# simplew4y/VeritasFi

Hardware: AMD Instinct MI355X
Metric: queries/sec top-100 over 10Mx768 corpus (higher is better)
Workload: dtype f16

## Files before the change

veritasfi_amd/csrc/vf_api.hip:

```cpp
#include "../../include/veritasfi_hip.h"
#include "vf_internal.h"
#include "vf_route.h"

#include <fcntl.h>
#include <float.h>
#include <sys/stat.h>
#include <unistd.h>
#include <math.h>
#include <string.h>

#include <algorithm>
#include <atomic>
#include <mutex>
#include <string>
#include <vector>

using namespace vf;

static thread_local std::string g_err;

static int fail(int code, const std::string& msg) {
    g_err = msg;
    return code;
}
// ... 40 lines not shown
        bytes = need;
        return VF_OK;
    }
    void release() { if (p) (void)hipFree(p); p = nullptr; bytes = 0; }
    template <class T> T* as() const { return (T*)p; }
};

struct HostBuf {
    void* p = nullptr;
    size_t bytes = 0;
    int ensure(size_t need) {
        if (need <= bytes) return VF_OK;
        if (p) { (void)hipHostFree(p); p = nullptr; bytes = 0; }
        hipError_t e = hipHostMalloc(&p, need, hipHostMallocDefault);
        if (e != hipSuccess) return fail(VF_ENOMEM, std::string("hipHostMalloc(") + std::to_string(need) + "): " + hipGetErrorString(e));
        bytes = need;
        return VF_OK;
    }
    void release() { if (p) (void)hipHostFree(p); p = nullptr; bytes = 0; }
};

struct Slot {
    hipStream_t stream = nullptr;
    hipStream_t scan_stream = nullptr;
    hipEvent_t ev_pro = nullptr;
    hipEvent_t ev_in = nullptr, ev_done = nullptr, ev_scan = nullptr;
    hipEvent_t ev_t[4] = {nullptr, nullptr, nullptr, nullptr};
    bool timed = false;
    int wide_launches = 0, wide_queries = 0;
    int scan_kernel = 0;
    int scan_image = 0;
    DevBuf qn, qimg, s0, cnt, tau, hist, hist_coarse, cand, flags, counts;
    DevBuf dbg, wgbase, tilecnt, sib;
    DevBuf qimg8, epsq;
    DevBuf qscale, bandq;
    int image_i8 = 0;
    int64_t wgbase_n = -1; int wgbase_grid = -1;
    DevBuf dense_s, cn_tmp, parts_ids, parts_sc, run_ids, run_sc, qsel;
    int* h_flags = nullptr;
    u32* h_counts = nullptr;
    int* d_flags = nullptr;
    u32* d_counts = nullptr;
    size_t h_cap = 0;
    bool pending = false;
    const float* d_queries = nullptr;
    int nq = 0, k = 0, path = 0;
    int64_t* d_ids = nullptr;
    float* d_scores = nullptr;
    hipStream_t user_stream = nullptr;
};

struct GroupSlot {
    std::vector<hipStream_t> feed;
    std::vector<hipEvent_t> ev;
    std::vector<DevBuf> dq, blob;
    DevBuf all;
    hipEvent_t ev_in = nullptr;
    hipStream_t hq_stream = nullptr;
    hipEvent_t ev_hq = nullptr;
    HostBuf hq;
    std::vector<hipStream_t> hfeed;
    std::vector<hipEvent_t> ev_hb;
    std::vector<hipEvent_t> ev_home;
    std::vector<HostBuf> hb;
    std::vector<char> staged_last;
    bool pending = false;
    int nq = 0, k = 0;
    int64_t* d_ids = nullptr; float* d_scores = nullptr;
    hipStream_t user = nullptr;
};

}

struct vf_index {
    int device = 0;
    int64_t n = 0;
    int64_t cap = 0;
    int d = 0, dp = 0, dtype = 0;
    int64_t id_offset = 0;
    int n_cu = 256;
    int64_t aux_applied = -1;
    bool owns_rows = false;
    void* rows_orig = nullptr;
    void* rows_scan = nullptr;
    bool owns_scan = false;
    float* norm = nullptr;
    float* inv_scan = nullptr;
    float* cn_cache = nullptr;
    unsigned char* rows_img = nullptr;
    bool owns_img = false;
    float* inv_img = nullptr;
    float rho_max = 0.0f;
    float rho_mean = 0.0f;
    bool image_refused = false;
    float rho_sum = 0.0f;
    std::mutex mu;
    Slot slots[kSlots];
    int64_t force_path = -1, sample_rows = -1, margin = -1, cap_opt = 0, waves_opt = 0, scan_g = 0,
            refresh_every = 128, debug = 0, steal_opt = 0, wide_opt = 1, wide_sync = -1, wide_mfma = -1, wide8_waves = 8, wide8_stage = 0,
            aux_cus = -1, sample_grid = -1, overlap_scans = -1, scan_impl = 2, sample_impl = -1, scan_image = 1, wide_rows = 1, image_mfma = -1;
    vf_search_stats stats{};
    bool profile = false;
    double prof_scan_ms = 0.0, prof_pipe_ms = 0.0;
    int64_t prof_launches = 0, prof_bytes = 0;
    hipEvent_t ev_span = nullptr;
    bool span_started = false;
    bool span_slot[4] = {false, false, false, false};
    DevBuf st_q, st_ids, st_sc;
    DevBuf st_add, st_rho;
    DevBuf st_cmp, st_rem;
    int64_t compact_chunk_rows = 0;
    int64_t subset_super_rows = 0;
    bool damaged = false;
    std::vector<vf_index*> shards;
    std::vector<int> peer_ok;
    GroupSlot gslots[kSlots];
};

static int ensure_pinned(Slot& s, size_t nq_total) {
    if (nq_total <= s.h_cap) return VF_OK;
    if (s.h_flags) (void)hipHostFree(s.h_flags);
    if (s.h_counts) (void)hipHostFree(s.h_counts);
    s.h_flags = nullptr; s.h_counts = nullptr; s.h_cap = 0;
    size_t cap = std::max<size_t>(nq_total, 256);
    VF_HIP(hipHostMalloc((void**)&s.h_flags, cap * sizeof(int), hipHostMallocMapped));
    VF_HIP(hipHostMalloc((void**)&s.h_counts, cap * sizeof(u32), hipHostMallocMapped));
    VF_HIP(hipHostGetDevicePointer((void**)&s.d_flags, s.h_flags, 0));
    VF_HIP(hipHostGetDevicePointer((void**)&s.d_counts, s.h_counts, 0));
    s.h_cap = cap;
    return VF_OK;
}

static int build_image(vf_index* ix, int64_t mode);
// ... 140 lines not shown
static void destroy_index(vf_index* ix) {
    if (!ix) return;
    if (!ix->shards.empty()) {
        for (int i = 0; i < kSlots; ++i) {
            GroupSlot& gs = ix->gslots[i];
            for (size_t g = 0; g < ix->shards.size(); ++g) {
                (void)hipSetDevice(ix->shards[g]->device);
                (void)hipDeviceSynchronize();
                if (g < gs.dq.size()) gs.dq[g].release();
                if (g < gs.blob.size()) gs.blob[g].release();
                if (g < gs.feed.size() && gs.feed[g]) (void)hipStreamDestroy(gs.feed[g]);
                if (g < gs.ev.size() && gs.ev[g]) (void)hipEventDestroy(gs.ev[g]);
                if (g < gs.ev_hb.size() && gs.ev_hb[g]) (void)hipEventDestroy(gs.ev_hb[g]);
                if (g < gs.hb.size()) gs.hb[g].release();
            }
            (void)hipSetDevice(ix->device);
            gs.all.release();
            gs.hq.release();
            for (hipStream_t st : gs.hfeed) if (st) (void)hipStreamDestroy(st);
            for (hipEvent_t ev : gs.ev_home) if (ev) (void)hipEventDestroy(ev);
            if (gs.hq_stream) (void)hipStreamDestroy(gs.hq_stream);
            if (gs.ev_hq) (void)hipEventDestroy(gs.ev_hq);
            if (gs.ev_in) (void)hipEventDestroy(gs.ev_in);
        }
        for (vf_index* sh : ix->shards) destroy_index(sh);
        ix->shards.clear();
    }
    (void)hipSetDevice(ix->device);
    (void)hipDeviceSynchronize();
    ix->st_q.release(); ix->st_ids.release(); ix->st_sc.release(); ix->st_add.release(); ix->st_rho.release(); ix->st_cmp.release(); ix->st_rem.release();
    for (int i = 0; i < kSlots; ++i) {
        Slot& s = ix->slots[i];
        DevBuf* bufs[] = {&s.qn, &s.qimg, &s.s0, &s.cnt, &s.tau, &s.hist, &s.hist_coarse, &s.cand, &s.flags, &s.counts, &s.dense_s,
                          &s.cn_tmp, &s.parts_ids, &s.parts_sc, &s.run_ids, &s.run_sc, &s.qsel, &s.dbg, &s.wgbase, &s.tilecnt, &s.sib};
        for (DevBuf* b : bufs) b->release();
        if (s.h_flags) (void)hipHostFree(s.h_flags);
        if (s.h_counts) (void)hipHostFree(s.h_counts);
        if (s.scan_stream && s.scan_stream != s.stream) (void)hipStreamDestroy(s.scan_stream);
        if (s.stream) (void)hipStreamDestroy(s.stream);
        if (s.ev_pro) (void)hipEventDestroy(s.ev_pro);
        if (s.ev_in) (void)hipEventDestroy(s.ev_in);
        if (s.ev_done) (void)hipEventDestroy(s.ev_done);
        if (s.ev_scan) (void)hipEventDestroy(s.ev_scan);
        for (int e = 0; e < 4; ++e) if (s.ev_t[e]) (void)hipEventDestroy(s.ev_t[e]);
    }
    if (ix->owns_scan && ix->rows_scan) (void)hipFree(ix->rows_scan);
    if (ix->owns_rows && ix->rows_orig) (void)hipFree(ix->rows_orig);
    if (ix->norm) (void)hipFree(ix->norm);
    if (ix->inv_scan) (void)hipFree(ix->inv_scan);
    if (ix->cn_cache) (void)hipFree(ix->cn_cache);
    if (ix->rows_img && ix->owns_img) (void)hipFree(ix->rows_img);
    if (ix->inv_img) (void)hipFree(ix->inv_img);
    if (ix->ev_span) (void)hipEventDestroy(ix->ev_span);
    delete ix;
}

static int create_impl(vf_index** out, const void* rows, bool rows_on_device, int64_t n, int32_t d, int32_t dtype,
                       int32_t device_id, int64_t id_offset, bool adopt = false) {
    if (!out) return fail(VF_EINVAL, "vf_index_create: null out");
    *out = nullptr;
    if (n < 0 || d <= 0 || (n > 0 && !rows)) return fail(VF_EINVAL, "vf_index_create: bad rows/n/d");
    if (!known_dtype(dtype)) return fail(VF_EINVAL, "vf_index_create: unknown dtype");
    if (n >= (int64_t)0xFFFFFFFFll) return fail(VF_EUNSUPPORTED, "vf_index_create: more than 2^32-1 rows per shard");
    int ndev = 0;
    VF_HIP(hipGetDeviceCount(&ndev));
    if (device_id < 0 || device_id >= ndev) return fail(VF_EINVAL, "vf_index_create: bad device_id");
    VF_HIP(hipSetDevice(device_id));
// ... 522 lines not shown
        if (ev[i]) (void)hipEventDestroy(ev[i]);
    }
    if (rc == VF_OK) {
        rc = create_impl(out, d_rows, true, n, (int32_t)h.d, (int32_t)h.dtype, device_id, id_offset, true);
        if (rc == VF_OK) { (*out)->owns_rows = true; d_rows = nullptr; }
    }
    if (d_rows) (void)hipFree(d_rows);
    return rc;
}

extern "C" int vf_index_destroy(vf_index* ix) {
    DeviceGuard restore_callers_device;
    if (!ix) return VF_OK;
    destroy_index(ix);
    return VF_OK;
}

extern "C" int vf_index_info(vf_index* ix, int64_t* n, int32_t* d, int32_t* dtype, int32_t* device_id) {
    if (!ix) return fail(VF_EINVAL, "vf_index_info: null handle");
    if (n) *n = ix->n;
    if (d) *d = ix->d;
    if (dtype) *dtype = ix->dtype;
    if (device_id) *device_id = ix->device;
    return VF_OK;
}

extern "C" int vf_index_stats(vf_index* ix, vf_search_stats* out) {
    if (!ix || !out) return fail(VF_EINVAL, "vf_index_stats: null argument");
    std::lock_guard<std::mutex> g(ix->mu);
    *out = ix->stats;
    return VF_OK;
}

extern "C" int vf_index_profile(vf_index* ix, double* scan_ms_total, int64_t* scan_launches, double* pipeline_ms_total,
                                int64_t* scan_bytes_per_launch) {
    if (!ix) return fail(VF_EINVAL, "vf_index_profile: null handle");
    std::lock_guard<std::mutex> g(ix->mu);
    double sm = ix->prof_scan_ms, pm = ix->prof_pipe_ms;
    int64_t nl = ix->prof_launches, nb = ix->prof_bytes;
    for (vf_index* sh : ix->shards) {
        std::lock_guard<std::mutex> lk(sh->mu);
        sm += sh->prof_scan_ms; pm += sh->prof_pipe_ms; nl += sh->prof_launches;
        if (nb == 0) nb = sh->prof_bytes;
    }
    if (scan_ms_total) *scan_ms_total = sm;
    if (scan_launches) *scan_launches = nl;
    if (pipeline_ms_total) *pipeline_ms_total = pm;
    if (scan_bytes_per_launch) *scan_bytes_per_launch = nb;
    return VF_OK;
}

extern "C" int vf_index_profile_span(vf_index* ix, double* span_ms, int64_t* launches) {
    if (!ix || !span_ms || !launches) return fail(VF_EINVAL, "vf_index_profile_span: null argument");
    DeviceGuard restore_callers_device;
    vf_index* t = ix->shards.empty() ? ix : ix->shards[0];
    std::lock_guard<std::mutex> g(t->mu);
    *span_ms = 0.0; *launches = t->prof_launches;
    if (!t->span_started || !t->ev_span) return VF_OK;
    VF_HIP(hipSetDevice(t->device));
    for (int i = 0; i < kSlots; ++i) {
        if (!t->span_slot[i] || !t->slots[i].ev_t[1] || t->slots[i].pending) continue;
        float ms = 0.f;
        if (hipEventElapsedTime(&ms, t->ev_span, t->slots[i].ev_t[1]) == hipSuccess && ms > *span_ms) *span_ms = ms;
        else (void)hipGetLastError();
    }
    return VF_OK;
// ... 42 lines not shown
        if (value != 8) return fail(VF_EINVAL, "wide8_waves must be 8 (the 4-wave form was measured slower and is built with -DVF_EXPERIMENTS only: DESIGN.md 4)");
#endif
        ix->wide8_waves = value;
    }
    else if (s == "wide_mfma") { if (!in_range(-1, 1)) return fail(VF_EINVAL, "wide_mfma must be -1 (auto: the fp8 instruction for e4m3 rows), 0 (fp16 matrix instruction on converted rows) or 1 (the fp8 instruction on the e4m3 row bytes: k_scan_wide8)"); ix->wide_mfma = value; }
    else if (s == "wide_sync") { if (!in_range(-1, 8)) return fail(VF_EINVAL, "wide_sync must be -1 (off) or a slack of 0..8 super-tiles"); ix->wide_sync = value; }
    else if (s == "aux_cus") {
        if (!in_range(-1, 128)) return fail(VF_EINVAL, "aux_cus must be -1 (auto) or in [0, 128]");
        if (ix->aux_applied >= 0 && value != ix->aux_cus)
            return fail(VF_EINVAL, "aux_cus is fixed once the first search has created the scan streams: set it before searching");
        ix->aux_cus = value;
    }
    else if (s == "sample_grid") { if (!in_range(-1, 1024)) return fail(VF_EINVAL, "sample_grid must be -1 (auto), 0 (one workgroup per range) or a workgroup count"); ix->sample_grid = value; }
    else if (s == "scan_impl") { if (!in_range(1, 5)) return fail(VF_EINVAL, "scan_impl must be 1 (k_scan), 2 (auto: k_scan2 for fp16 rows, k_scan2r where it measured faster), 3 (k_scan2 wherever it fits, e4m3 rows converted), 4 (k_scan2 for fp16 rows, never k_scan2r) or 5 (k_scan2r wherever a shape of it exists: fp16 rows of 384 / 512 / 768 / 1024 elements, e4m3 rows of 768 / 1024)"); ix->scan_impl = value; }
    else if (s == "sample_impl") { if (!in_range(-1, 1)) return fail(VF_EINVAL, "sample_impl must be -1 (auto: k_scan2r's operand path for the sample pass where it exists and the CU split is on), 0 (k_scan) or 1 (k_scan2r wherever it fits)"); ix->sample_impl = value; }
    else if (s == "overlap_scans") { if (!in_range(-1, 1)) return fail(VF_EINVAL, "overlap_scans must be -1 (auto), 0 or 1"); ix->overlap_scans = value; }
    else if (s == "scan_image") {
        if (!in_range(0, 2)) return fail(VF_EINVAL, "scan_image must be 0 (off), 1 (auto: when it fits with headroom) or 2 (force)");
        if (ix->damaged) return fail(VF_EHIP, std::string("scan_image: ") + kDamagedMsg);
        if (!ix->shards.empty()) { ix->scan_image = value; return VF_OK; }
        for (const Slot& sl : ix->slots) if (sl.pending) return fail(VF_EINVAL, "scan_image cannot change while a search is pending");
        DeviceGuard restore_callers_device;
        VF_HIP(hipSetDevice(ix->device));
        VF_HIP(hipDeviceSynchronize());
        ix->image_refused = false;
        if (value == 0) free_image(ix);
        else VF_TRY(build_image(ix, value));
        ix->scan_image = value;
    }
    else if (s == "image_mfma") { if (!in_range(-1, 2)) return fail(VF_EINVAL, "image_mfma must be -1 (auto), 0 (the int8 row image on the fp16 matrix instruction, fp16 queries), 1 (on the int8 matrix instruction, the queries as one int8 plane) or 2 (as two planes, hi + lo: the band of 0)"); ix->image_mfma = value; }
    else if (s == "wide_rows") { if (!in_range(0, 2)) return fail(VF_EINVAL, std::string("wide_rows must be 0 (rows of more than 2432 padded elements never take the fused path), 1 (auto: from ") + std::to_string(kWideRowsMinRows) + " rows, e4m3 rows from " + std::to_string(kWideRowsMinRows8) + ", int8 rows from " + std::to_string(kWideRowsMinRowsI8) + ") or 2 (wherever k_scan_ksplit / k_scan_ksplit8 serve them; int8 rows: from " + std::to_string(kWideRowsMinRowsI8) + " rows)"); ix->wide_rows = value; }
    else if (s == "compact_chunk_rows") { if (!in_range(0, kMaxShardRows)) return fail(VF_EINVAL, "compact_chunk_rows must be 0 (auto: 64 MB of staging) or the destination rows a removal moves per chunk"); ix->compact_chunk_rows = value; }
    else if (s == "subset_super_rows") { if (!in_range(0, kSubsetMaxRows)) return fail(VF_EINVAL, "subset_super_rows must be 0 (auto: 64 MB of scores) or the listed rows a subset search scores per launch"); ix->subset_super_rows = value; }
    else if (s == "debug") ix->debug = value;
    else if (s == "profile") {
        ix->profile = value != 0; ix->prof_scan_ms = ix->prof_pipe_ms = 0.0; ix->prof_launches = 0;
        ix->span_started = false;
        for (bool& b : ix->span_slot) b = false;
    }
    else return fail(VF_EINVAL, "vf_index_set_option: unknown option " + s);
    return VF_OK;
}

static int exact_search(vf_index* ix, Slot& s, const float* qn_dev, int nq, int k, int64_t* out_ids,
                        float* out_scores, hipStream_t st) {
    const int dt = ix->dtype;
    const int64_t chunk = kSmallN;
    const int64_t nchunks = ix->n == 0 ? 1 : (ix->n + chunk - 1) / chunk;
    if (nchunks > 1) {
        int64_t P = 1;
        while (P < 2 * (int64_t)k) P <<= 1;
        if (P * 8 > 160 * 1024) return fail(VF_EUNSUPPORTED, "exact chunked search supports k <= 8192 when n > 16384");
    }
    VF_TRY(s.dense_s.ensure((size_t)nq * chunk * sizeof(float)));
    if (nchunks == 1) {
        const float* cn = ix->cn_cache;
        if (!cn && ix->n > 0) {
            VF_TRY(s.cn_tmp.ensure((size_t)chunk * ix->d * sizeof(float)));
            VF_HIP(launch_normalize_rows(ix->rows_orig, dt, 0, ix->n, ix->d, ix->norm, s.cn_tmp.as<float>(), st));
            cn = s.cn_tmp.as<float>();
        }
        VF_HIP(launch_dense_dot16(qn_dev, nq, cn, ix->n, ix->d, s.dense_s.as<float>(), chunk, st));
        VF_HIP(launch_sort_rows(s.dense_s.as<float>(), chunk, nq, (int)ix->n, k, ix->id_offset, (long long*)out_ids,
                                out_scores, k, st));
        return VF_OK;
    }
// ... 186 lines not shown
    s.timed = ix->profile;
    if (s.timed) VF_HIP(hipEventRecord(s.ev_t[2], st));
    if (s.wgbase_n != ix->n || s.wgbase_grid != p.grid) {
        std::vector<long long> base(p.grid);
        for (int w = 0; w < p.grid; ++w) base[w] = ix->n * (long long)w / p.grid;
        VF_TRY(s.wgbase.ensure((size_t)p.grid * sizeof(long long)));
        VF_HIP(hipMemcpy(s.wgbase.p, base.data(), (size_t)p.grid * sizeof(long long), hipMemcpyHostToDevice));
        s.wgbase_n = ix->n; s.wgbase_grid = p.grid;
    }
    for (int b0 = 0; b0 < nq; b0 += bl) {
        const int nb = std::min(bl, nq - b0);
        const BatchRoute b = route_batch(in, r, nb);
        const int qt = b.tile;
        float* qn_b = s.qn.as<float>() + (size_t)b0 * ix->d;
        VF_HIP(launch_prep_queries(d_queries + (size_t)b0 * ix->d, nb, ix->d, ix->dp, qt, qn_b, s.image_i8 ? nullptr : s.qimg.as<_Float16>(), st));
        ScanArgs a{};
        a.rows = (const char*)ix->rows_scan; a.inv_scan = ix->inv_scan; a.qimg = s.qimg.as<_Float16>();
        if (s.image_i8) {
            VF_TRY(s.qimg8.ensure((size_t)ix->dp * kMaxBatch * 2));
            VF_TRY(s.epsq.ensure(kMaxBatch * sizeof(float)));
            VF_TRY(s.qscale.ensure(kMaxBatch * sizeof(float)));
            VF_TRY(s.bandq.ensure(2 * kMaxBatch * sizeof(int)));
            VF_HIP(launch_prep_q8(qn_b, nb, ix->d, ix->dp, qt, s.image_i8, (signed char*)s.qimg8.p, s.qscale.as<float>(), s.epsq.as<float>(), s.bandq.as<int>(),
                                  p.eps, p.tau_band, p.fine_band, st));
            a.qimg = (const _Float16*)s.qimg8.p; a.q_scale = s.qscale.as<float>(); a.band_q = s.bandq.as<int>();
        }
        a.n = ix->n; a.dp = ix->dp; a.row_bytes = (long long)ix->dp * (byte_rows(ix->dtype) ? 1 : 2); a.total_waves = p.total_waves; a.samp = p.samp;
        if (p.image) { a.rows = (const char*)ix->rows_img; a.inv_scan = ix->inv_img; a.off_scan = image_offsets(ix); a.row_bytes = ix->dp; }
        a.s0 = s.s0.as<float>(); a.wg_base = s.wgbase.as<long long>(); a.cnt = s.cnt.as<u32>(); a.tau_bin = s.tau.as<int>(); a.hist = s.hist.as<u32>();
        a.cand = s.cand.as<u64>(); a.cap = p.cap; a.kprime = p.kprime; a.tau_band = p.tau_band;
        a.hist_coarse = s.hist_coarse.as<u32>(); a.stage_cap = b.stage_cap;
        a.tile_cnt = ix->steal_opt ? s.tilecnt.as<u32>() : nullptr; a.scan_grid = p.grid;
        a.dbg = nullptr;
        if (ix->debug & 128) { VF_TRY(s.dbg.ensure((size_t)p.total_waves * ((ix->debug & 512) ? 72 : 4) * sizeof(u64))); a.dbg = s.dbg.as<u64>(); if (ix->debug & 512) VF_HIP(hipMemsetAsync(s.dbg.p, 0, s.dbg.bytes, st)); }
        a.refresh_every = (int)std::min<int64_t>(256, std::max<int64_t>(4, std::max<int64_t>(1, ix->refresh_every) * nb / kMaxBatch));
        while (a.refresh_every & (a.refresh_every - 1)) a.refresh_every &= a.refresh_every - 1;
        a.nq = nb; a.debug = (int)ix->debug;
        if (ix->n / p.total_waves < p.samp)
            VF_HIP(hipMemsetAsync(a.s0, 0xFF, (size_t)qt * p.total_waves * p.samp * sizeof(float), st));
        switch (b.sample) {
        case kKernelKsplit: VF_HIP(launch_scan_ksplit(a, kModeSample, b.sample_grid, st)); break;
        case kKernelKsplit8: VF_HIP(launch_scan_ksplit8(a, kModeSample, b.sample_grid, b.sample_rows, st)); break;
        case kKernelScan2r: {
            ScanArgs as = a;
            as.stage_cap = 0;
            VF_HIP(launch_scan2r_sample(as, qt, b.sample_grid, b.sample_rows, st));
            break;
        }
        default: VF_HIP(launch_scan(a, kModeSample, qt, b.sample_grid, (int)ix->scan_g, b.sample_rows, st));
        }
        VF_HIP(launch_sel0(a, qt, st));
        hipStream_t sst = s.scan_stream;
        if (sst != st) {
            VF_HIP(hipEventRecord(s.ev_pro, st));
            VF_HIP(hipStreamWaitEvent(sst, s.ev_pro, 0));
        }
        if (!route_overlap(in))
            for (int o = 0; o < kSlots; ++o)
                if (o != slot_id && ix->slots[o].ev_scan) VF_HIP(hipStreamWaitEvent(sst, ix->slots[o].ev_scan, 0));
        if (s.timed && b0 == 0) {
            if (!ix->span_started) {
                if (!ix->ev_span) VF_HIP(hipEventCreate(&ix->ev_span));
                VF_HIP(hipEventRecord(ix->ev_span, sst));
                ix->span_started = true;
            }
            ix->span_slot[slot_id] = true;
// ... 997 lines not shown
```

veritasfi_amd/csrc/vf_internal.h:

```cpp
#pragma once
#include <hip/hip_runtime.h>
#include <math.h>
#include <stdint.h>

#include "../../include/veritasfi_hip.h"

#include <string>

#include "vf_ksplit_geom.h"
#include "vf_compact.h"
#include "vf_subset.h"

namespace vf {

int set_error(int code, const std::string& msg);

typedef unsigned long long u64;
typedef unsigned int u32;

struct DeviceGuard {
    int prev = -1;
    DeviceGuard() { if (hipGetDevice(&prev) != hipSuccess) prev = -1; }
    ~DeviceGuard() { if (prev >= 0) (void)hipSetDevice(prev); }
    DeviceGuard(const DeviceGuard&) = delete;
// ... 30 lines not shown
__host__ __device__ inline Q8Bound image_q8_bound(float rho_q) {
    Q8Bound b;
    if (!(rho_q < 1.0f)) { b.eps_add = INFINITY; b.tau_bins = kHistBins; b.fine_bins = 16 * kHistBins; return b; }
    const double c = (double)rho_q * (65.0 / 64.0);
    b.eps_add = (float)c;
    if ((double)b.eps_add < c) b.eps_add = nextafterf(b.eps_add, INFINITY);
    b.tau_bins = (int)ceil(c * (kHistBins / 2));
    b.fine_bins = (int)ceil(c * (kHistBins / 2) * 16);
    return b;
}
__host__ __device__ inline float image_q8_eps(float eps_img, float eps_add) {
    const float e = nextafterf(eps_img + eps_add, INFINITY) + 0x1p-20f;
    return nextafterf(e, INFINITY);
}

struct ScanArgs {
    const char* rows;
    const float* inv_scan;
    const float* off_scan;
    const float* q_scale;
    const _Float16* qimg;
    long long n;
    int dp;
    long long row_bytes;
    int total_waves;
    int samp;
    float* s0;
    const long long* wg_base;
    u32* cnt;
    int* tau_bin;
    u32* hist;
    u32* hist_coarse;
    int stage_cap;
    u64* cand;
    int cap;
    int kprime;
    int tau_band;
    const int* band_q;
    int refresh_every;
    int nq;
    u32* tile_cnt;
    int scan_grid;
    int qn_total, jtiles, rgroups;
    u32* sib;
    int sib_slack;
    unsigned long long* dbg;
    int debug;
};

struct FinalArgs {
    const u32* cnt; const u64* cand; int cap;
    int top_cap, sel_cap;
    const int* tau_bin;
    const void* rows_orig; int orig_dtype; long long orig_row_elems;
    const float* norm;
    const float* qn;
    int d; int k; int kprime; float eps;
    const float* eps_q;
    int band;
    const int* band_q;
    long long n_rows;
    long long id_offset;
    long long* out_ids; float* out_scores;
    int* flags;
    u32* cand_count_out;
    unsigned long long* dbg;
// ... 81 lines not shown
```

veritasfi_amd/csrc/vf_kernels.hip:

```cpp
#include "vf_internal.h"

#include <float.h>
#include <algorithm>
#include <type_traits>

#include <mutex>

namespace vf {

typedef _Float16 h8 __attribute__((ext_vector_type(8)));
typedef _Float16 h4 __attribute__((ext_vector_type(4)));
typedef float f16v __attribute__((ext_vector_type(16)));
typedef int i4v __attribute__((ext_vector_type(4)));
typedef int i16v __attribute__((ext_vector_type(16)));
typedef int i8v __attribute__((ext_vector_type(8)));

__device__ __forceinline__ float group16_tree(float acc) {
    acc = acc + __shfl_down(acc, 8, 16);
    acc = acc + __shfl_down(acc, 4, 16);
    acc = acc + __shfl_down(acc, 2, 16);
    acc = acc + __shfl_down(acc, 1, 16);
    return acc;
}

// ... 889 lines not shown
    float off_lane = 0.0f;
};

#define VF_DPP_ROR(v, n) (u32) __builtin_amdgcn_update_dpp(0, (int)(v), 0x120 + (n), 0xF, 0xF, false)
__device__ __forceinline__ u32 wave_or_u32(u32 v) {
    v |= VF_DPP_ROR(v, 1);
    v |= VF_DPP_ROR(v, 2);
    v |= VF_DPP_ROR(v, 4);
    v |= VF_DPP_ROR(v, 8);
    return (u32)(__builtin_amdgcn_readlane((int)v, 0) | __builtin_amdgcn_readlane((int)v, 16) |
                 __builtin_amdgcn_readlane((int)v, 32) | __builtin_amdgcn_readlane((int)v, 48));
}
__device__ __forceinline__ u32 wave_sum_u32(u32 v) {
    v += VF_DPP_ROR(v, 1);
    v += VF_DPP_ROR(v, 2);
    v += VF_DPP_ROR(v, 4);
    v += VF_DPP_ROR(v, 8);
    return (u32)(__builtin_amdgcn_readlane((int)v, 0) + __builtin_amdgcn_readlane((int)v, 16) +
                 __builtin_amdgcn_readlane((int)v, 32) + __builtin_amdgcn_readlane((int)v, 48));
}

template <int NT, int MODE>
__device__ __forceinline__ void epi_prefetch(EpiRegs<NT>& e, const ScanArgs& a, long long t0, int lane, bool sync_tau) {
    e.inv_lane = a.inv_scan[t0 + (lane & 31)];
    e.sync_tau = sync_tau;
    if (MODE == kModeMain && sync_tau) {
#pragma unroll
        for (int nt = 0; nt < NT; ++nt)
            e.tau_g[nt] = __hip_atomic_load(a.tau_bin + nt * kQueryTile + (lane & 31), __ATOMIC_RELAXED,
                                            __HIP_MEMORY_SCOPE_AGENT);
    }
}

template <int NT, int MODE, bool PUBLISH = true, bool INV_LDS = false, bool OFF = false>
__device__ __forceinline__ void tile_epilogue(const ScanArgs& a, const f16v (&acc)[NT], const EpiRegs<NT>& e,
                                              long long t0, long long hi, long long s0_slot, int lane, char* ctl) {
    const int r31 = lane & 31, h = lane >> 5;
    auto inv_of = [&](int reg) {
        const int r0 = (reg & 3) + 8 * (reg >> 2);
        const float lo_half = __builtin_bit_cast(float, __builtin_amdgcn_readlane(__builtin_bit_cast(int, e.inv_lane), r0));
        const float hi_half = __builtin_bit_cast(float, __builtin_amdgcn_readlane(__builtin_bit_cast(int, e.inv_lane), r0 + 4));
        return h ? hi_half : lo_half;
    };
    auto off_of = [&](int reg) {
        const int r0 = (reg & 3) + 8 * (reg >> 2);
        const float lo_half = __builtin_bit_cast(float, __builtin_amdgcn_readlane(__builtin_bit_cast(int, e.off_lane), r0));
        const float hi_half = __builtin_bit_cast(float, __builtin_amdgcn_readlane(__builtin_bit_cast(int, e.off_lane), r0 + 4));
        return h ? hi_half : lo_half;
    };
    if (MODE == kModeSample) {
        const long long s0_stride = (long long)a.total_waves * a.samp;
#pragma unroll
        for (int nt = 0; nt < NT; ++nt) {
            const int q = nt * kQueryTile + r31;
#pragma unroll
            for (int reg = 0; reg < 16; ++reg) {
                const int rr = (reg & 3) + 8 * (reg >> 2) + 4 * h;
                if constexpr (OFF) {
                    if (t0 + rr < hi) a.s0[(long long)q * s0_stride + s0_slot + rr] = acc[nt][reg] * inv_of(reg) + off_of(reg);
                } else {
                    if (t0 + rr < hi) a.s0[(long long)q * s0_stride + s0_slot + rr] = acc[nt][reg] * inv_of(reg);
                }
            }
        }
        return;
    }
    int* tau_lds = (int*)(ctl + 16);
// ... 61 lines not shown
            umask |= m;
            total += (u32)__popc(m);
        }
    } else {
        umask = wave_or_u32(mask);
        total = wave_sum_u32((u32)__popc(mask));
    }
    u32* stage_cnt = (u32*)ctl;
    uint4* stage_ent = (uint4*)(ctl + kCtlBytes);
    const u32 rs = 31u - (u32)__builtin_clz((u32)a.refresh_every | 1u);
    const u32 R = 1u << rs;
    u32 base = 0;
    if (lane == 0) base = atomicAdd(stage_cnt, total);
    base = (u32)__builtin_amdgcn_readfirstlane((int)base);
    const bool need = (base >> rs) != ((base + total) >> rs);
    if (a.debug & 8) return;
    u32 run = base;
    const u32 edge = (((base + total) >> rs) << rs) - 1u;
    int qq = 0;
    for (u32 um = umask; um != 0u; um &= um - 1u) {
        const int pair = __builtin_ctz(um);
        const int nt = pair >> 4, reg = pair & 15;
        const int q = nt * kQueryTile + r31;
        const bool mine = ((mask >> pair) & 1u) != 0u;
        const unsigned long long bal = __ballot(mine);
        if (mine) {
            const u32 slot = run + __builtin_amdgcn_mbcnt_hi((u32)(bal >> 32), __builtin_amdgcn_mbcnt_lo((u32)bal, 0u));
            const int rr = (reg & 3) + 8 * (reg >> 2) + 4 * h;
            const float sc = m[pair];
            const u32 bin = (u32)bin_of_x(bin_x(sc));
            const u32 key = orderkey(sc), row = (u32)(t0 + rr);
            if (slot < (u32)a.stage_cap) {
                stage_ent[slot] = make_uint4(row, key, (u32)q | (bin << 8), 1u);
            } else {
                const u32 gs = atomicAdd(a.cnt + q * kCntStride, 1u);
                if (gs < (u32)a.cap) a.cand[(long long)q * a.cap + gs] = ((u64)key << 32) | (u64)row;
                atomicAdd(a.hist + (long long)q * kHistBins + bin, 1u);
                atomicAdd(a.hist_coarse + q * 64 + (bin >> 5), 1u);
            }
        }
        const u32 nxt = run + (u32)__popcll(bal);
        if (run <= edge && edge < nxt) qq = nt * kQueryTile + ((__ffsll((long long)bal) - 1) & 31);
        run = nxt;
    }
    if (a.debug & 2) return;
    if constexpr (!PUBLISH) return;
    if (need) {
        const int nb = wave_tau_two_level(a.hist_coarse + qq * 64, a.hist + (long long)qq * kHistBins, a.kprime, lane) - (a.band_q ? a.band_q[qq] : a.tau_band);
        if (lane == 0 && nb > 0) {
            atomicMax(a.tau_bin + qq, nb);
            atomicMax(tau_lds + qq, nb);
        }
        for (u32 blk = base >> rs; blk < (base + total) >> rs; ++blk)
        for (u32 j = (u32)lane; j < R; j += 64u) {
            const u32 idx = (blk << rs) + j;
            if (idx >= (u32)a.stage_cap) break;
            const uint4 en = stage_ent[idx];
            if (en.w == 1u) {
                const u32 q = en.z & 0xFFu, bin = en.z >> 8;
                if (q < (u32)QN_of<NT>() && bin < (u32)kHistBins) {
                    atomicAdd(a.hist + (long long)q * kHistBins + bin, 1u);
                    atomicAdd(a.hist_coarse + q * 64 + (bin >> 5), 1u);
                }
            }
        }
    }
// ... 1104 lines not shown
                }
                buf = buf + 1 == RING ? 0 : buf + 1;
                VF_PC(pt1 = cyc(); pc_fill += pt1 - pt0)
            };
#define VF_R_SEG(N) if constexpr (RB > N) { consume(std::integral_constant<int, N>{}, nullptr); refill(N); }
            VF_R_SEG(0) VF_R_SEG(1) VF_R_SEG(2) VF_R_SEG(3) VF_R_SEG(4) VF_R_SEG(5)
#undef VF_R_SEG
            for (int sg = RB; sg < S; ++sg) {
                consume(std::integral_constant<int, -1>{}, lds_lane + (long long)(sg - RB) * SEGIMG);
                refill(sg);
            }
            VF_PC(pt0 = cyc())
            const char* sc = scratch + (tiles_done & 1) * 512;
            EpiRegs<NT> epi;
            epi.inv_lane = *(const float*)(sc + 256 + r31 * 4);
            epi.inv_lds = sc + 256;
            if constexpr (F8 >= 2) epi.off_lane = *(const float*)(sc + 384 + r31 * 4);
            if constexpr (I8) {
#pragma unroll
                for (int nt = 0; nt < NT; ++nt)
#pragma unroll
                    for (int e = 0; e < 16; ++e) {
                        float v = (float)acci[0][nt][e];
                        if constexpr (PLANES == 2) { v = v * 254.0f + (float)acci[1][nt][e]; acci[1][nt][e] = 0; }
                        acc[nt][e] = v * sq[nt];
                        acci[0][nt][e] = 0;
                    }
            }
            epi.sync_tau = sync_now;
            if (sync_now) {
#pragma unroll
                for (int nt = 0; nt < NT; ++nt) epi.tau_g[nt] = *(const int*)(sc + (nt * kQueryTile + r31) * 4);
            }
            tile_epilogue<NT, MODE, true, true, F8 >= 2>(a, acc, epi, t0, t_hi, t_s0, lane, ctl);
#pragma unroll
            for (int nt = 0; nt < NT; ++nt)
#pragma unroll
                for (int e = 0; e < 16; ++e) acc[nt][e] = 0.0f;
            VF_PC(pt1 = cyc(); pc_epi += pt1 - pt0)
            ++tiles_done;
            if (!more) break;
            cur_tile = nxt;
            src_cur = src_nxt;
        }
    }
    if (dbg && dbg_rec > 4) dbg[69] = (unsigned long long)tiles_done;
    asm volatile("s_waitcnt vmcnt(0)" ::: "memory");
    if (MODE == kModeSample) return;
    if (lane == 0) atomicAdd((u32*)(ctl + 8), 1u);
    if (dbg) dbg[1] = wall_clock64();
    __syncthreads();
    if (dbg) dbg[2] = wall_clock64();
    {
        const u32 staged = *(const u32*)ctl;
        const u32 nst = staged < (u32)a.stage_cap ? staged : (u32)a.stage_cap;
        uint4* ent = (uint4*)(ctl + kCtlBytes);
        u32* qcnt = (u32*)(kImgBytes ? img : smem);
        u32* qbase = qcnt + QN;
        if (tid < QN) qcnt[tid] = 0u;
        __syncthreads();
        for (u32 i = tid; i < nst; i += THREADS) {
            const uint4 e = ent[i];
            const u32 q = e.z & 0xFFu;
            if (e.w != 1u || q >= (u32)QN) continue;
            ent[i].w = 2u + atomicAdd(qcnt + q, 1u);
        }
        __syncthreads();
        if (tid < QN) {
            const u32 c = qcnt[tid];
            qbase[tid] = c ? atomicAdd(a.cnt + tid * kCntStride, c) : 0u;
        }
        __syncthreads();
        for (u32 i = tid; i < nst; i += THREADS) {
            const uint4 e = ent[i];
            if (e.w < 2u) continue;
            const u32 q = e.z & 0xFFu;
            const u32 gs = qbase[q] + (e.w - 2u);
            if (gs < (u32)a.cap) a.cand[(long long)q * a.cap + gs] = ((u64)e.y << 32) | (u64)e.x;
        }
    }
    if (dbg && dbg_rec > 4) dbg[71] = __builtin_amdgcn_s_memtime() - c_entry;
#ifdef VF_EXPERIMENTS
    if (dbg && dbg_rec > 4 && prof) { dbg[4] = pc_wait; dbg[5] = pc_use; dbg[6] = pc_fill; dbg[7] = pc_head; dbg[8] = pc_epi; dbg[9] = pc_n; }
#endif
#undef VF_PC
    if (dbg) dbg[3] = wall_clock64();
}

constexpr int kWideNT = kWideQ / kQueryTile, kWideRows = 256;
#ifndef VF_WIDE_THREADS
#define VF_WIDE_THREADS 512
#endif
constexpr int kWideThreads = VF_WIDE_THREADS, kWideWaves = kWideThreads / 64, kWideM = kWideRows / kWideWaves / kRowTile;
constexpr int kSampWaves = kScanThreads / 64;

template <int F8> struct WideStage { uint4 w[kWideM][4]; };
template <int F8> __device__ __forceinline__ constexpr int wide_dc() { return F8 ? 2 : 1; }

template <int F8>
__device__ __forceinline__ void wide_issue_a(WideStage<F8>& st, const char* rows, long long row_bytes, const long long (&row)[kWideM],
                                             int unit, int h) {
#pragma unroll
    for (int m = 0; m < kWideM; ++m) {
        if constexpr (F8 != 0) {
            const char* p = rows + row[m] * row_bytes + (long long)unit * 128 + h * 32;
            st.w[m][0] = *(const uint4*)p;
            st.w[m][1] = *(const uint4*)(p + 16);
            st.w[m][2] = *(const uint4*)(p + 64);
            st.w[m][3] = *(const uint4*)(p + 80);
        } else {
            const char* p = rows + row[m] * row_bytes + (long long)unit * 128 + h * 64;
// ... 1181 lines not shown
    auto emit = [&](float x, long long i) {
        if (x > -INFINITY && bin_of_x(bin_x(x)) >= tb) {
            const u32 slot = atomicAdd(&lcnt, 1u);
            const u32 wg = (u32)i / (u32)swg;
            const long long row = a.wg_base[wg] + (long long)((u32)i - wg * (u32)swg);
            if (slot < (u32)a.cap) a.cand[(long long)q * a.cap + slot] = ((u64)orderkey(x) << 32) | (u64)(u32)row;
        }
    };
    if (q < a.nq) {
        if (in_regs) {
#pragma unroll
            for (int u = 0; u < kKeep; ++u) emit(v[u], tid + (long long)u * 1024);
        } else {
            for (long long i = tid; i < len; i += 1024) emit(s[i], i);
        }
    }
    __syncthreads();
    for (int b = tid; b < kHistBins; b += 1024) a.hist[(long long)q * kHistBins + b] = (q < a.nq && b >= tb) ? lh[b] : 0u;
    if (tid < 64) {
        u32 c = 0;
#pragma unroll
        for (int i = 0; i < 32; ++i) {
            const int b = tid * 32 + i;
            c += (q < a.nq && b >= tb) ? lh[b] : 0u;
        }
        a.hist_coarse[q * 64 + tid] = c;
    }
    if (tid == 0) {
        a.cnt[q * kCntStride] = lcnt;
        a.tau_bin[q] = (q < a.nq && !(a.debug & 1)) ? tb : kHistBins;
    }
    if (q == 0 && a.tile_cnt)
        for (int i = tid; i < a.scan_grid; i += 1024) a.tile_cnt[i] = 0u;
}

hipError_t launch_sel0(const ScanArgs& a, int qn_tile, hipStream_t s) {
    hipLaunchKernelGGL(k_sel0, dim3(qn_tile), dim3(1024), 0, s, a);
    return hipGetLastError();
}

constexpr int kFinalThreads = 256;

__device__ __forceinline__ void rank_select_desc(const u64* keys, int n, u64* out, int limit, int tid) {
    for (int i0 = tid; i0 < n; i0 += 4 * kFinalThreads) {
        u64 mine[4];
        int rank[4];
#pragma unroll
        for (int u = 0; u < 4; ++u) {
            const int i = i0 + u * kFinalThreads;
            mine[u] = i < n ? keys[i] : 0ull;
            rank[u] = 0;
        }
        int j = 0;
        for (; j + 16 <= n; j += 16) {
            u64 kj[16];
#pragma unroll
            for (int t = 0; t < 16; ++t) kj[t] = keys[j + t];
#pragma unroll
            for (int t = 0; t < 16; ++t)
#pragma unroll
                for (int u = 0; u < 4; ++u) rank[u] += kj[t] > mine[u] ? 1 : 0;
        }
        for (; j < n; ++j) {
            const u64 kj = keys[j];
#pragma unroll
            for (int u = 0; u < 4; ++u) rank[u] += kj > mine[u] ? 1 : 0;
// ... 499 lines not shown
```

veritasfi_amd/csrc/vf_scan_lds.h:

```cpp
#pragma once
#include <stddef.h>

#if defined(__HIPCC__)
#define VF_HD __host__ __device__ __forceinline__
#else
#define VF_HD inline
#endif

namespace vf {

constexpr int kQueryTile = 32;
constexpr int kMaxBatch = 64;
constexpr int kRowTile = 32;
constexpr int kScanThreads = 512;
constexpr int kHistBins = 2048;
constexpr int kSmallN = 16384;
constexpr int kMaxCap = 8192;
constexpr int kCntStride = 32;
constexpr int kMaxKFused = 2048;

constexpr int kLdsBytes = 160 * 1024;
constexpr int kStageMaxBytes = 32 * 1024;
constexpr int kStageMinEntries = 256;

// ... 23 lines not shown
    return img + (size_t)kScan2Waves * (kRing * kSegBytes + kScratchBytes) + kCtlBytes + (size_t)stage_cap * 16;
}
VF_HD int scan2_stage_cap(int dp, int qn_tile, RowForm rows) {
    const size_t fixed = scan2_lds_bytes(dp, qn_tile, 0);
    if ((dp >> (rows ? 7 : 6)) < kRing) return 0;
    if (fixed + kStageMinEntries * 16 > (size_t)kLdsBytes) return 0;
    return stage_entries(fixed);
}

struct Scan2rShape { int S, RB, RING; };
VF_HD Scan2rShape scan2r_shape(int dp, RowForm f8) {
    if (!f8 && dp == 768) return {12, 6, 6};
    if (!f8 && dp == 1024) return {16, 6, 4};
    if (!f8 && dp == 512) return {8, 4, 6};
    if (!f8 && dp == 384) return {6, 3, 6};
    if (f8 == kRowsI8Mfma1) return dp == 768 ? Scan2rShape{6, 6, 6} : Scan2rShape{0, 0, 0};
    if (f8 == kRowsI8Mfma2) return dp == 768 ? Scan2rShape{6, 3, 6} : Scan2rShape{0, 0, 0};
    if (f8 && dp == 768) return {6, 3, 6};
    if (f8 && dp == 1024) return {8, 3, 4};
    return {0, 0, 0};
}
VF_HD size_t scan2r_lds_bytes(int dp, int qn_tile, int stage_cap, RowForm f8) {
    const Scan2rShape sh = scan2r_shape(dp, f8);
    const size_t seg_img = (size_t)(f8 ? 128 : 64) * qn_tile * 2;
    return (size_t)(sh.S - sh.RB) * seg_img + (size_t)kScan2Waves * (sh.RING * kSegBytes + kScratchBytes) + kCtlBytes + (size_t)stage_cap * 16;
}
VF_HD int scan2r_stage_cap(int dp, int qn_tile, RowForm f8) {
    if (scan2r_shape(dp, f8).S == 0) return 0;
    const size_t fixed = scan2r_lds_bytes(dp, qn_tile, 0, f8);
    if (fixed + kStageMinEntries * 16 > (size_t)kLdsBytes) return 0;
    return stage_entries(fixed);
}

constexpr int kWideQ = 256, kWideKC = 64;
constexpr int kWideBuf = (kWideKC / 8) * kWideQ * 16;
constexpr int kWideCtl = 16 + 3 * kWideQ * 4;
constexpr int kWideStageCap = 3584;

VF_HD size_t scan_wide_lds_bytes(int stage_cap) { return (size_t)3 * kWideBuf + kWideCtl + (size_t)stage_cap * 16; }
VF_HD size_t scan_wide8_lds_bytes(int waves, int stage_cap) {
    return waves == 8 ? scan_wide_lds_bytes(stage_cap) : (size_t)65536 + (16 + 3 * 128 * 4) + (size_t)stage_cap * 16;
}
VF_HD int scan_wide8_stage_cap(int waves) { return waves == 8 ? kWideStageCap : 896; }

}
```

Before: 49320.

## Add per-workgroup global spill area for k_scan2r stage overflow

When the LDS stage of k_scan2r fills, candidates are now written to a per-workgroup spill buffer in global memory instead of doing a per-candidate global atomic on the list counter. At the end of the tile they are read back in stage-sized chunks and flushed through the same batched per-query counter reservation used for staged entries. The goal is fewer contended global atomics on overflow. The cost is extra global writes and reads, plus histogram atomics for each spilled entry. Tier counters and a debug API are added.

```diff
diff --git a/veritasfi_amd/csrc/vf_api.hip b/veritasfi_amd/csrc/vf_api.hip
--- a/veritasfi_amd/csrc/vf_api.hip
+++ b/veritasfi_amd/csrc/vf_api.hip
@@ -96,6 +96,7 @@
     int scan_image = 0;
     DevBuf qn, qimg, s0, cnt, tau, hist, hist_coarse, cand, flags, counts;
     DevBuf dbg, wgbase, tilecnt, sib;
+    DevBuf spill, tiers;
     DevBuf qimg8, epsq;
     DevBuf qscale, bandq;
     int image_i8 = 0;
@@ -162,7 +163,7 @@
     Slot slots[kSlots];
     int64_t force_path = -1, sample_rows = -1, margin = -1, cap_opt = 0, waves_opt = 0, scan_g = 0,
             refresh_every = 128, debug = 0, steal_opt = 0, wide_opt = 1, wide_sync = -1, wide_mfma = -1, wide8_waves = 8, wide8_stage = 0,
-            aux_cus = -1, sample_grid = -1, overlap_scans = -1, scan_impl = 2, sample_impl = -1, scan_image = 1, wide_rows = 1, image_mfma = -1;
+            aux_cus = -1, sample_grid = -1, overlap_scans = -1, scan_impl = 2, sample_impl = -1, scan_image = 1, wide_rows = 1, image_mfma = -1, spill_cap = -1;
     vf_search_stats stats{};
     bool profile = false;
     double prof_scan_ms = 0.0, prof_pipe_ms = 0.0;
@@ -369,7 +370,7 @@
     for (int i = 0; i < kSlots; ++i) {
         Slot& s = ix->slots[i];
         DevBuf* bufs[] = {&s.qn, &s.qimg, &s.s0, &s.cnt, &s.tau, &s.hist, &s.hist_coarse, &s.cand, &s.flags, &s.counts, &s.dense_s,
-                          &s.cn_tmp, &s.parts_ids, &s.parts_sc, &s.run_ids, &s.run_sc, &s.qsel, &s.dbg, &s.wgbase, &s.tilecnt, &s.sib};
+                          &s.cn_tmp, &s.parts_ids, &s.parts_sc, &s.run_ids, &s.run_sc, &s.qsel, &s.dbg, &s.wgbase, &s.tilecnt, &s.sib, &s.spill, &s.tiers};
         for (DevBuf* b : bufs) b->release();
         if (s.h_flags) (void)hipHostFree(s.h_flags);
         if (s.h_counts) (void)hipHostFree(s.h_counts);
@@ -958,6 +959,19 @@
     return VF_OK;
 }
 
+extern "C" int vf_debug_scan_tiers(vf_index* ix, int32_t slot, int64_t* staged, int64_t* spilled, int64_t* direct) {
+    DeviceGuard restore_callers_device;
+    if (!ix || !staged || !spilled || !direct || slot < 0 || slot >= kSlots) return fail(VF_EINVAL, "vf_debug_scan_tiers: bad argument");
+    std::lock_guard<std::mutex> g(ix->mu);
+    const Slot& s = ix->slots[slot];
+    if (s.pending || s.scan_kernel != kKernelScan2r || !s.tiers.p) return fail(VF_EINVAL, "vf_debug_scan_tiers: the slot's last search is pending or did not run k_scan2r");
+    VF_HIP(hipSetDevice(ix->device));
+    u64 t[3];
+    VF_HIP(hipMemcpy(t, s.tiers.p, sizeof t, hipMemcpyDeviceToHost));
+    *staged = (int64_t)t[0]; *spilled = (int64_t)t[1]; *direct = (int64_t)t[2];
+    return VF_OK;
+}
+
 extern "C" int vf_index_profile(vf_index* ix, double* scan_ms_total, int64_t* scan_launches, double* pipeline_ms_total,
                                 int64_t* scan_bytes_per_launch) {
     if (!ix) return fail(VF_EINVAL, "vf_index_profile: null handle");
@@ -1066,6 +1080,7 @@
     else if (s == "wide_rows") { if (!in_range(0, 2)) return fail(VF_EINVAL, std::string("wide_rows must be 0 (rows of more than 2432 padded elements never take the fused path), 1 (auto: from ") + std::to_string(kWideRowsMinRows) + " rows, e4m3 rows from " + std::to_string(kWideRowsMinRows8) + ", int8 rows from " + std::to_string(kWideRowsMinRowsI8) + ") or 2 (wherever k_scan_ksplit / k_scan_ksplit8 serve them; int8 rows: from " + std::to_string(kWideRowsMinRowsI8) + " rows)"); ix->wide_rows = value; }
     else if (s == "compact_chunk_rows") { if (!in_range(0, kMaxShardRows)) return fail(VF_EINVAL, "compact_chunk_rows must be 0 (auto: 64 MB of staging) or the destination rows a removal moves per chunk"); ix->compact_chunk_rows = value; }
     else if (s == "subset_super_rows") { if (!in_range(0, kSubsetMaxRows)) return fail(VF_EINVAL, "subset_super_rows must be 0 (auto: 64 MB of scores) or the listed rows a subset search scores per launch"); ix->subset_super_rows = value; }
+    else if (s == "spill_cap") { if (!in_range(-1, 1 << 21)) return fail(VF_EINVAL, "spill_cap must be -1 (auto: scan2r_spill_cap), 0 (no spill area: a full stage appends to the lists directly) or the entries per workgroup of k_scan2r's spill area"); ix->spill_cap = value; }
     else if (s == "debug") ix->debug = value;
     else if (s == "profile") {
         ix->profile = value != 0; ix->prof_scan_ms = ix->prof_pipe_ms = 0.0; ix->prof_launches = 0;
@@ -1318,6 +1333,12 @@
         a.hist_coarse = s.hist_coarse.as<u32>(); a.stage_cap = b.stage_cap;
         a.tile_cnt = ix->steal_opt ? s.tilecnt.as<u32>() : nullptr; a.scan_grid = p.grid;
         a.dbg = nullptr;
+        if (b.main == kKernelScan2r) {
+            a.spill_cap = scan2r_spill_cap(b.stage_cap, p.grid, (long long)kMaxBatch * p.cap, ix->spill_cap);
+            if (a.spill_cap > 0) { VF_TRY(s.spill.ensure((size_t)p.grid * a.spill_cap * sizeof(uint4))); a.spill = s.spill.as<uint4>(); }
+            VF_TRY(s.tiers.ensure(3 * sizeof(u64)));
+            a.tiers = s.tiers.as<u64>(); a.tiers_reset = b0 == 0;
+        }
         if (ix->debug & 128) { VF_TRY(s.dbg.ensure((size_t)p.total_waves * ((ix->debug & 512) ? 72 : 4) * sizeof(u64))); a.dbg = s.dbg.as<u64>(); if (ix->debug & 512) VF_HIP(hipMemsetAsync(s.dbg.p, 0, s.dbg.bytes, st)); }
         a.refresh_every = (int)std::min<int64_t>(256, std::max<int64_t>(4, std::max<int64_t>(1, ix->refresh_every) * nb / kMaxBatch));
         while (a.refresh_every & (a.refresh_every - 1)) a.refresh_every &= a.refresh_every - 1;
diff --git a/veritasfi_amd/csrc/vf_internal.h b/veritasfi_amd/csrc/vf_internal.h
--- a/veritasfi_amd/csrc/vf_internal.h
+++ b/veritasfi_amd/csrc/vf_internal.h
@@ -86,6 +86,10 @@
     u32* hist;
     u32* hist_coarse;
     int stage_cap;
+    uint4* spill;
+    int spill_cap;
+    unsigned long long* tiers;
+    int tiers_reset;
     u64* cand;
     int cap;
     int kprime;
diff --git a/veritasfi_amd/csrc/vf_kernels.hip b/veritasfi_amd/csrc/vf_kernels.hip
--- a/veritasfi_amd/csrc/vf_kernels.hip
+++ b/veritasfi_amd/csrc/vf_kernels.hip
@@ -945,7 +945,7 @@
     }
 }
 
-template <int NT, int MODE, bool PUBLISH = true, bool INV_LDS = false, bool OFF = false>
+template <int NT, int MODE, bool PUBLISH = true, bool INV_LDS = false, bool OFF = false, bool SPILL = false>
 __device__ __forceinline__ void tile_epilogue(const ScanArgs& a, const f16v (&acc)[NT], const EpiRegs<NT>& e,
                                               long long t0, long long hi, long long s0_slot, int lane, char* ctl) {
     const int r31 = lane & 31, h = lane >> 5;
@@ -1073,6 +1073,10 @@
             const u32 key = orderkey(sc), row = (u32)(t0 + rr);
             if (slot < (u32)a.stage_cap) {
                 stage_ent[slot] = make_uint4(row, key, (u32)q | (bin << 8), 1u);
+            } else if (SPILL && a.spill && slot - (u32)a.stage_cap < (u32)a.spill_cap) {
+                a.spill[(size_t)blockIdx.x * (size_t)a.spill_cap + (slot - (u32)a.stage_cap)] = make_uint4(row, key, (u32)q | (bin << 8), 1u);
+                atomicAdd(a.hist + (long long)q * kHistBins + bin, 1u);
+                atomicAdd(a.hist_coarse + q * 64 + (bin >> 5), 1u);
             } else {
                 const u32 gs = atomicAdd(a.cnt + q * kCntStride, 1u);
                 if (gs < (u32)a.cap) a.cand[(long long)q * a.cap + gs] = ((u64)key << 32) | (u64)row;
@@ -2243,7 +2247,7 @@
 #pragma unroll
                 for (int nt = 0; nt < NT; ++nt) epi.tau_g[nt] = *(const int*)(sc + (nt * kQueryTile + r31) * 4);
             }
-            tile_epilogue<NT, MODE, true, true, F8 >= 2>(a, acc, epi, t0, t_hi, t_s0, lane, ctl);
+            tile_epilogue<NT, MODE, true, true, F8 >= 2, MODE == kModeMain>(a, acc, epi, t0, t_hi, t_s0, lane, ctl);
 #pragma unroll
             for (int nt = 0; nt < NT; ++nt)
 #pragma unroll
@@ -2268,26 +2272,49 @@
         uint4* ent = (uint4*)(ctl + kCtlBytes);
         u32* qcnt = (u32*)(kImgBytes ? img : smem);
         u32* qbase = qcnt + QN;
-        if (tid < QN) qcnt[tid] = 0u;
-        __syncthreads();
-        for (u32 i = tid; i < nst; i += THREADS) {
-            const uint4 e = ent[i];
-            const u32 q = e.z & 0xFFu;
-            if (e.w != 1u || q >= (u32)QN) continue;
-            ent[i].w = 2u + atomicAdd(qcnt + q, 1u);
-        }
-        __syncthreads();
-        if (tid < QN) {
-            const u32 c = qcnt[tid];
-            qbase[tid] = c ? atomicAdd(a.cnt + tid * kCntStride, c) : 0u;
-        }
-        __syncthreads();
-        for (u32 i = tid; i < nst; i += THREADS) {
-            const uint4 e = ent[i];
-            if (e.w < 2u) continue;
-            const u32 q = e.z & 0xFFu;
-            const u32 gs = qbase[q] + (e.w - 2u);
-            if (gs < (u32)a.cap) a.cand[(long long)q * a.cap + gs] = ((u64)e.y << 32) | (u64)e.x;
+        auto flush_pass = [&](u32 cnt) {
+            if (tid < QN) qcnt[tid] = 0u;
+            __syncthreads();
+            for (u32 i = tid; i < cnt; i += THREADS) {
+                const uint4 e = ent[i];
+                const u32 q = e.z & 0xFFu;
+                if (e.w != 1u || q >= (u32)QN) continue;
+                ent[i].w = 2u + atomicAdd(qcnt + q, 1u);
+            }
+            __syncthreads();
+            if (tid < QN) {
+                const u32 c = qcnt[tid];
+                qbase[tid] = c ? atomicAdd(a.cnt + tid * kCntStride, c) : 0u;
+            }
+            __syncthreads();
+            for (u32 i = tid; i < cnt; i += THREADS) {
+                const uint4 e = ent[i];
+                if (e.w < 2u) continue;
+                const u32 q = e.z & 0xFFu;
+                const u32 gs = qbase[q] + (e.w - 2u);
+                if (gs < (u32)a.cap) a.cand[(long long)q * a.cap + gs] = ((u64)e.y << 32) | (u64)e.x;
+            }
+        };
+        flush_pass(nst);
+        u32 nsp = 0;
+        if (a.spill && staged > (u32)a.stage_cap && !(a.debug & 8)) nsp = staged - (u32)a.stage_cap < (u32)a.spill_cap ? staged - (u32)a.stage_cap : (u32)a.spill_cap;
+        const u64* strip = (const u64*)(a.spill + (size_t)blockIdx.x * (size_t)a.spill_cap);
+        for (u32 c0 = 0; c0 < nsp; c0 += (u32)a.stage_cap) {
+            const u32 m = nsp - c0 < (u32)a.stage_cap ? nsp - c0 : (u32)a.stage_cap;
+            __syncthreads();
+            for (u32 i = tid; i < m; i += THREADS) {
+                const u64 rk = __hip_atomic_load(strip + 2 * (size_t)(c0 + i), __ATOMIC_RELAXED, __HIP_MEMORY_SCOPE_AGENT);
+                const u64 qb = __hip_atomic_load(strip + 2 * (size_t)(c0 + i) + 1, __ATOMIC_RELAXED, __HIP_MEMORY_SCOPE_AGENT);
+                ent[i] = make_uint4((u32)rk, (u32)(rk >> 32), (u32)qb, 1u);
+            }
+            __syncthreads();
+            flush_pass(m);
+        }
+        if (a.tiers && tid == 0) {
+            const u32 over = staged - nst - nsp;
+            if (nst) atomicAdd(a.tiers, (unsigned long long)nst);
+            if (nsp) atomicAdd(a.tiers + 1, (unsigned long long)nsp);
+            if (over) atomicAdd(a.tiers + 2, (unsigned long long)over);
         }
     }
     if (dbg && dbg_rec > 4) dbg[71] = __builtin_amdgcn_s_memtime() - c_entry;
@@ -3535,6 +3562,7 @@
     }
     if (q == 0 && a.tile_cnt)
         for (int i = tid; i < a.scan_grid; i += 1024) a.tile_cnt[i] = 0u;
+    if (q == 0 && a.tiers && a.tiers_reset && tid < 3) a.tiers[tid] = 0ull;
 }
 
 hipError_t launch_sel0(const ScanArgs& a, int qn_tile, hipStream_t s) {
diff --git a/veritasfi_amd/csrc/vf_scan_lds.h b/veritasfi_amd/csrc/vf_scan_lds.h
--- a/veritasfi_amd/csrc/vf_scan_lds.h
+++ b/veritasfi_amd/csrc/vf_scan_lds.h
@@ -79,6 +79,17 @@
     return stage_entries(fixed);
 }
 
+constexpr int kSpillStride = kScan2Waves * 64;
+constexpr long long kSpillMaxBytes = 32ll * 1024 * 1024;
+VF_HD int scan2r_spill_cap(int stage_cap, int grid, long long list_entries, long long opt) {
+    if (opt == 0 || grid <= 0 || stage_cap <= 0) return 0;
+    const long long lim = kSpillMaxBytes / 16 / grid / kSpillStride * kSpillStride;
+    long long want = opt > 0 ? opt : (list_entries + grid - 1) / grid - stage_cap;
+    if (want < 0) want = 0;
+    want = (want + kSpillStride - 1) / kSpillStride * kSpillStride;
+    return (int)(want < lim ? want : lim);
+}
+
 constexpr int kWideQ = 256, kWideKC = 64;
 constexpr int kWideBuf = (kWideKC / 8) * kWideQ * 16;
 constexpr int kWideCtl = 16 + 3 * kWideQ * 4;
```

Result: slower. 47520 (-3.7%).
